# thourihan/DeepfakeDetection

Hardware: AMD Instinct MI355X
Metric: train images/sec @224^2 (EfficientNet-B0) (higher is better)
Workload: dtype bf16; 1 GPU; EfficientNet-b0 (timm flavour) 224x224 train step: bf16 fwd + label-smoothed CE + bwd + AdamW, random-init weights, 2 classes; per_gpu_batch=256, global_batch=256, parallelism=dp1, launch=hipgraph

## Files before the change

deepfakedetection_amd/_lib.py:

```python

from __future__ import annotations

import ctypes
from ctypes import POINTER, Structure, c_double, c_float, c_int, c_int64, c_long, c_size_t, c_uint32, c_void_p
from pathlib import Path

import os as _os

LIB_PATH = Path(_os.environ.get("DFD_LIB_PATH") or Path(__file__).resolve().parent / "libdfd_hip.so")

DFD_OK = 0
ERRORS = {-1: "DFD_EINVAL", -2: "DFD_EUNSUPPORTED", -3: "DFD_ELAUNCH", -4: "DFD_EWORKSPACE"}
F32, BF16 = 0, 1
ACT_NONE, ACT_SILU, ACT_RELU, ACT_GELU = 0, 1, 2, 3
PRO_NONE, PRO_BN_ACT, PRO_BN_ACT_GATE, PRO_AFFINE2 = 0, 1, 2, 3
MAX_PARTIALS = 1024
ADAMW_TABLE_COLS = 5
ADAMW_HP_LEN = 8
EMA_TABLE_COLS = 4
EMA_LERP, EMA_COPY = 0, 1
MIX_JOB_WORDS = 8
MIX_KEEP, MIX_MIXUP, MIX_CUTMIX = 0, 1, 2
MIX_NHWC, MIX_NCHW = 0, 1
AUG_MAX_OPS = 4
# ... 63 lines not shown
    "dfd_pwconv_bwd_fused": (c_int, [c_int, P, P, P, P, P, P, c_int, c_int, c_int, P, P, c_int, P, c_size_t, P]),
    "dfd_pw_prep_weights": (c_int, [c_int, P, P, P, c_int, c_int, P]),
    "dfd_stem_conv_fwd": (c_int, [c_int, P, P, P, POINTER(StemShape), P, c_int, _PI, P]),
    "dfd_stem_conv_wgrad": (c_int, [c_int, P, P, P, P, P, POINTER(StemShape), c_int, P, c_size_t, P]),
    "dfd_stem_conv_wgrad_ws": (c_size_t, [POINTER(StemShape)]),
    "dfd_dropout": (c_int, [P, P, c_float, P, c_int, P]),
    "dfd_linear_fwd": (c_int, [P, P, P, P, c_int, c_int, c_int, P]),
    "dfd_linear_bwd": (c_int, [P, P, P, P, P, P, c_int, c_int, c_int, c_int, P]),
    "dfd_ce_loss": (c_int, [P, P, c_int, c_int, c_float, c_float, P, P, P, P]),
    "dfd_softmax_argmax": (c_int, [P, c_int, c_int, P, P, P]),
    "dfd_adamw_step": (c_int, [P, c_int, P, P]),
    "dfd_ema_update": (c_int, [P, c_int, P, P]),
    "dfd_mix_batch": (c_int, [P, P, P, P, c_int, c_int, c_int, c_int, c_int, P]),
    "dfd_ce_loss_soft": (c_int, [P, P, c_int, c_int, c_float, c_float, P, P, P, P]),
    "dfd_augment_policy_u8": (c_int, [P, P, P, P, c_int, c_int, c_int, P]),
    "dfd_bn_eval_coeffs_multi": (c_int, [P, c_int, P]),
    "dfd_sum_batch_begin": (c_int, []),
    "dfd_sum_batch_end": (c_int, []),
    "dfd_sum_batch_end_deferred": (c_int, []),
    "dfd_sum_passengers_flush": (c_int, [P]),
    "dfd_sum_passengers_discard": (c_int, []),
    "dfd_se_fwd": (c_int, [c_int, P, P, c_int, c_int, c_int, c_int, P, P, P, P, c_int, c_int, P, P, P, P, P, c_size_t, P]),
    "dfd_se_bwd": (c_int, [c_int, P, P, P, c_int, c_int, c_int, c_int, P, P, P, P, P, c_int, c_int, P, P, P, P, P, P, c_int,
                           P, c_size_t, P, P]),
    "dfd_pwconv_fwd_eval": (c_int, [c_int, P, P, P, c_int, P, c_int, c_int, c_int, P]),
    "dfd_dwconv_fwd_eval_tiles": (c_int, [c_int, P]),
    "dfd_dwconv_fwd_eval": (c_int, [c_int, P, P, P, c_int, P, P, P, P, P]),
    "dfd_se_fwd_parts": (c_int, [P, c_int, c_int, c_int, c_int, P, P, P, P, c_int, c_int, P, P, P, P, P]),
    "dfd_bn_finalize_ex": (c_int, [P, c_int, c_int, c_double, P, P, P, P, P, P, c_float, c_float, P, P]),
    "dfd_bn_eval_coeffs_ex": (c_int, [P, P, P, P, P, P, c_float, c_int, P, P]),
# ... 120 lines not shown
```

deepfakedetection_amd/build.py:

```python

from __future__ import annotations

import os
import shutil
import subprocess
import sys
from concurrent.futures import ThreadPoolExecutor
from pathlib import Path

PKG_DIR = Path(__file__).resolve().parent
CSRC = PKG_DIR / "csrc"
OBJ_DIR = CSRC / "build"
LIB_PATH = PKG_DIR / "libdfd_hip.so"
SOURCES = ("dfd_rowpass.hip", "dfd_dwfwd.hip", "dfd_dwbwd.hip", "dfd_dwbwdf.hip", "dfd_dwconv.hip", "dfd_dwmm.hip", "dfd_pwconv.hip", "dfd_pwntw.hip", "dfd_pwntd.hip", "dfd_pwtnw.hip", "dfd_misc.hip", "dfd_vit.hip",
           "dfd_mx.hip", "dfd_attn.hip", "dfd_coord.hip", "dfd_resize.hip", "dfd_augment.hip", "dfd_conv3.hip", "dfd_stem.hip", "dfd_gemm.hip", "dfd_cam.hip", "dfd_mix.hip")
ARCH = "gfx950"
FLAGS = ("-O3", "-fPIC", "-std=c++17", "-ffp-contract=off", f"--offload-arch={ARCH}")


def _hipcc() -> str:
    found = shutil.which("hipcc") or "/opt/rocm/bin/hipcc"
    if not Path(found).exists():
        raise RuntimeError("hipcc not found: libdfd_hip.so cannot be built")
    return found


def _deps_mtime() -> float:
    headers = list(CSRC.glob("*.h")) + [PKG_DIR.parent / "include" / "dfd_hip.h"]
    return max(p.stat().st_mtime for p in headers)
# ... 49 lines not shown
```

deepfakedetection_amd/csrc/dfd_common.h:

```cpp
#pragma once
#include <hip/hip_runtime.h>
#include <stdint.h>
#include <mutex>
#include "../../include/dfd_hip.h"

#define DFD_THREADS 256

template <typename Tag, typename KernelT>
static inline void dfd_allow_lds_once(KernelT kern, int bytes) {
    static std::once_flag once;
    std::call_once(once, [&] { (void)hipFuncSetAttribute(reinterpret_cast<const void*>(kern), hipFuncAttributeMaxDynamicSharedMemorySize, bytes); });
}
template <typename Tag, typename KernelT>
static inline int dfd_kernel_regs_once(KernelT kern, int fallback) {
    static std::once_flag once;
    static int regs = 0;
    std::call_once(once, [&] {
        hipFuncAttributes attr;
        regs = (hipFuncGetAttributes(&attr, reinterpret_cast<const void*>(kern)) == hipSuccess && attr.numRegs > 0) ? attr.numRegs : fallback;
    });
    return regs;
}

struct bf16 { unsigned short x; };
// ... 203 lines not shown
int dfd_stem_wgrad_mfma(const float* x, const void* dz, const void* yraw, const float* coef, const dfd_stem_shape* s, float* ws,
                        int max_rows, int* rows, hipStream_t st);

#define DFD_CHECK_LAUNCH() (hipGetLastError() == hipSuccess ? DFD_OK : DFD_ELAUNCH)

#define DISPATCH_ACT(ACTV, ...)                                                      \
    switch (ACTV) {                                                                  \
        case DFD_ACT_NONE: { constexpr int ACT = DFD_ACT_NONE; __VA_ARGS__; } break; \
        case DFD_ACT_SILU: { constexpr int ACT = DFD_ACT_SILU; __VA_ARGS__; } break; \
        case DFD_ACT_RELU: { constexpr int ACT = DFD_ACT_RELU; __VA_ARGS__; } break; \
        case DFD_ACT_GELU: { constexpr int ACT = DFD_ACT_GELU; __VA_ARGS__; } break; \
        default: return DFD_EUNSUPPORTED;                                            \
    }

enum { DFD_TUNE_DW_MFMA = 0, DFD_TUNE_DW_LDS_KB = 1, DFD_TUNE_DW_GRID = 2, DFD_TUNE_DEBUG = 3, DFD_TUNE_PW_NTD = 4, DFD_TUNE_NTD_NS = 5, DFD_TUNE_NTD_MAXN = 6, DFD_TUNE_NTD_MINT = 7,
       DFD_TUNE_DWQ_GRID_FWD = 8, DFD_TUNE_DWQ_GRID_BWD = 9, DFD_TUNE_DWQ_GRID_WGRAD = 10, DFD_TUNE_DWQ_GRID_MIN = 11, DFD_TUNE_TN_WGS = 12, DFD_TUNE_DWQ_WIDE = 13,
       DFD_TUNE_COUNT = 16 };
int dfd_tune_get(int key);

int dfd_launch_sum_partials(float* partials, int P, long L, float* out, int accumulate, hipStream_t st, bool deferrable = true);
```

deepfakedetection_amd/csrc/dfd_dwmm.hip:

```cpp
#include "dfd_dwm.h"
#include <climits>

typedef float dwm_f4 __attribute__((ext_vector_type(4)));
typedef __bf16 dwm_bf8 __attribute__((ext_vector_type(8)));

static int g_tune[DFD_TUNE_COUNT] = { 1,  156,  256,  0,  1,  0,  0,  16,
                                       1024,  1024,  1024,  32,  512,  -1};
int dfd_tune_get(int key) { return (key >= 0 && key < DFD_TUNE_COUNT) ? g_tune[key] : 0; }
extern "C" int dfd_tune(int key, int value) {
    if (key < 0 || key >= DFD_TUNE_COUNT) return DFD_EINVAL;
    g_tune[key] = value;
    return DFD_OK;
}

#define DWP_THREADS 512
#define DWP_MAXV 6
#define DWP_MAXS 4
#define DWP_MAXR 8

template <int K, int S, int ACT, bool PRO, bool STATS, bool WHOLE>
__global__ void __launch_bounds__(DWP_THREADS, 2)
k_dw_fwd_mp(const unsigned short* __restrict__ x, const float* __restrict__ bnstate, const float* __restrict__ w,
            unsigned short* __restrict__ y, DwMGeom g, float* __restrict__ partials, int dbg) {
    constexpr int KK = K * K, NPAIR = (KK + 1) / 2;
// ... 415 lines not shown
```

deepfakedetection_amd/csrc/dfd_misc.hip:

```cpp
#include "dfd_common.h"
#include "dfd_se.h"

__device__ __forceinline__ float wave_sum(float v) {
#pragma unroll
    for (int o = 32; o >= 1; o >>= 1) v += __shfl_xor(v, o);
    return v;
}
__device__ __forceinline__ float wave_max(float v) {
#pragma unroll
    for (int o = 32; o >= 1; o >>= 1) v = fmaxf(v, __shfl_xor(v, o));
    return v;
}
template <int ACT> __device__ __forceinline__ float act_rt(float z) { return act_fwd<ACT>(z); }

#define SE_MAX_C 4096
#define SE_MAX_R 128

__device__ __forceinline__ float wave_dot(const float* __restrict__ a, const float* __restrict__ b, int C, int lane) {
    float s = 0.f;
    for (int c = lane * 4; c < C; c += 256) {
        const float4 x = *reinterpret_cast<const float4*>(a + c);
        const float4 y = *reinterpret_cast<const float4*>(b + c);
        s = fmaf(x.x, y.x, fmaf(x.y, y.y, fmaf(x.z, y.z, fmaf(x.w, y.w, s))));
    }
// ... 266 lines not shown
                          const float* gate, const float* hpre, const float* pooled, const float* w1, const float* w2t, int R,
                          int act, float* dgate, float* dpooled, float* dw1, float* db1, float* dw2, float* db2, int accumulate,
                          void* pool_ws, size_t pool_ws_bytes, float* ws, dfd_stream stream) {
    if (!D || !y || !bnstate || !gate || !hpre || !pooled || !w1 || !w2t || !dgate || !dpooled || !ws || N < 1 || C < 1 ||
        R < 1 || C % 4)
        return DFD_EINVAL;
    if (C > SE_MAX_C || R > SE_MAX_R) return DFD_EUNSUPPORTED;
    hipStream_t st = (hipStream_t)stream;
    int splits = 1;
    float mul = 1.f;
    const int rc = dfd_pool_launch(dtype, true, D, y, bnstate, act_in, dgate, N, HW, C, pool_ws, pool_ws_bytes, st, &splits, &mul);
    if (rc != DFD_OK) return rc;
    DISPATCH_ACT(act, {
        hipLaunchKernelGGL((k_se_bwd_img<ACT>), dim3(N), dim3(SE_IMG_THREADS), 0, st, (const float*)pool_ws, splits, dgate, gate, hpre,
                           w1, w2t, N, C, R, ws, dpooled);
    });
    if (hipGetLastError() != hipSuccess) return DFD_ELAUNCH;
    if (dw1 && dw2) {
        hipLaunchKernelGGL(k_se_fc_bwd_w, dim3((C + 63) / 64, R), dim3(DFD_THREADS), 0, st, pooled, ws, N, C, R, dw1, db1,
                           dw2, db2, accumulate);
    }
    return DFD_CHECK_LAUNCH();
}

extern "C" int dfd_se_fc_bwd(const float* dgate, const float* gate, const float* hpre, const float* pooled,
                             const float* w1, const float* w2t, int N, int C, int R, int act, float* dpooled,
                             float* dw1, float* db1, float* dw2, float* db2, int accumulate, float* ws,
                             dfd_stream stream) {
    if (!dgate || !gate || !hpre || !pooled || !w1 || !w2t || !dpooled || !ws || N < 1 || C < 1 || R < 1) return DFD_EINVAL;
    if (C > SE_MAX_C || R > SE_MAX_R) return DFD_EUNSUPPORTED;
// ... 670 lines not shown
```

deepfakedetection_amd/csrc/dfd_rowpass.hip:

```cpp
#include "dfd_common.h"
#include "dfd_se.h"
#include "dfd_sum.h"

template <typename T, int ACT, bool HAS_RES, bool HAS_RS>
__global__ void __launch_bounds__(DFD_THREADS)
k_bn_act_apply(const T* __restrict__ y, const float* __restrict__ bnstate, const T* __restrict__ res,
               const float* __restrict__ rs, T* __restrict__ out, long total_vec, int CV, int C, long vec_per_img) {
    constexpr int V = Vec<T>::N;
    const long stride = (long)gridDim.x * DFD_THREADS;
    const long first = (long)blockIdx.x * DFD_THREADS + threadIdx.x;
    int cv = (int)(first % CV);
    const int cstep = (int)(stride % CV);
    for (long i = first; i < total_vec; i += stride, cv = cv + cstep >= CV ? cv + cstep - CV : cv + cstep) {
        const int c0 = cv * V;
        float v[V], sc[V], sh[V];
        Vec<T>::load(y + i * V, v);
        load_f32<V>(bnstate + c0, sc);
        load_f32<V>(bnstate + C + c0, sh);
        float r = 1.f;
        if constexpr (HAS_RS) r = rs[i / vec_per_img];
        float q[V];
        if constexpr (HAS_RES) Vec<T>::load(res + i * V, q);
        bn_act_array<ACT, V>(v, sc, sh);
#pragma unroll
// ... 75 lines not shown
                if constexpr (HAS_Y) acc[V + j] += gg * (yv[j] - mean[j]) * rstd[j];
            }
        }
    }
    reduce_rowlanes<2 * V>(acc, red, cm.cvb, cm.rpb, vl, rl, active);
    if (rl == 0) {
        float* p = partials + (long)blockIdx.x * (HAS_Y ? 2 : 1) * C;
        float a0[V], a1[V];
#pragma unroll
        for (int j = 0; j < V; ++j) { a0[j] = acc[j]; a1[j] = acc[V + j]; }
        store_f32<V>(p + c0, a0);
        if constexpr (HAS_Y) store_f32<V>(p + C + c0, a1);
    }
}

struct SeWgradJob { const float* pooled; const float* ws; int N, C, R; float* dw1; float* db1; float* dw2; float* db2; int accumulate; };

template <typename T, int ACT, int MODE>
__global__ void __launch_bounds__(DFD_THREADS)
k_act_bn_bwd(const T* __restrict__ D, const T* __restrict__ y, const float* __restrict__ gate,
             const float* __restrict__ dpool, const float* __restrict__ bnstate, T* __restrict__ dz,
             long rows, int HW, int C, float invHW, ChanMap cm, float* __restrict__ partials, int main_x, SeWgradJob job,
             SumJobs sum1, SumJobs sum2) {
    constexpr int V = Vec<T>::N;
    __shared__ float red[DFD_THREADS * 2 * V];
    if ((int)blockIdx.x >= main_x) {
        int id = ((int)blockIdx.x - main_x) * (int)gridDim.y + (int)blockIdx.y;
        const int cb = (job.C + 63) / 64, nse = job.dw1 ? cb * job.R : 0;
        if (id < nse) {
            se_fc_bwd_w_body(job.pooled, job.ws, job.N, job.C, job.R, job.dw1, job.db1, job.dw2, job.db2, job.accumulate, id % cb, id / cb, red);
            return;
// ... 561 lines not shown
                                      dfd_stream stream) {
    if (!partials || nparts < 1 || C < 1 || count <= 0 || !bnstate || !coef) return DFD_EINVAL;
    if (dls && (!ls_gamma || !beta)) return DFD_EINVAL;
    const int threads = FIN_CH * FIN_LANES, grid = (C + FIN_CH - 1) / FIN_CH;
    hipLaunchKernelGGL(k_bn_bwd_finalize, dim3(grid), dim3(threads), 0, (hipStream_t)stream, partials, nparts, C, count,
                       gamma, beta, ls_gamma, bnstate, train, dgamma, dbeta, dls, dbias, accumulate, coef);
    return DFD_CHECK_LAUNCH();
}
extern "C" int dfd_bn_bwd_finalize(const float* partials, int nparts, int C, double count, const float* gamma,
                                   const float* bnstate, int train, float* dgamma, float* dbeta, int accumulate,
                                   float* coef, dfd_stream stream) {
    return dfd_bn_bwd_finalize_ex(partials, nparts, C, count, gamma, nullptr, nullptr, bnstate, train, dgamma, dbeta, nullptr,
                                  nullptr, accumulate, coef, stream);
}

extern "C" int dfd_version(void) { return 139; }
```

deepfakedetection_amd/csrc/dfd_se.h:

```cpp
#pragma once
#include "dfd_common.h"

__device__ __forceinline__ float se_wave_sum(float v) {
#pragma unroll
    for (int o = 32; o > 0; o >>= 1) v += __shfl_xor(v, o);
    return v;
}

__device__ __forceinline__ void se_fc_bwd_w_body(const float* __restrict__ pooled, const float* __restrict__ ws, int N, int C, int R,
                                                 float* __restrict__ dw1, float* __restrict__ db1, float* __restrict__ dw2,
                                                 float* __restrict__ db2, int accumulate, int bx, int by, float* red) {
    const float* ws_g = ws;
    const float* ws_dh = ws + (long)N * C;
    const float* ws_h = ws_dh + (long)N * R;
    const int t = threadIdx.x, cl = t & 63, nl = t >> 6;
    const int c = bx * 64 + cl, r = by;
    float a1 = 0.f, a2 = 0.f, sb2 = 0.f;
    if (c < C) {
        int n = nl;
        for (; n + 12 < N; n += 16) {
            float g[4], pc[4], h[4], dh[4];
#pragma unroll
            for (int u = 0; u < 4; ++u) {
                const long m = n + 4 * u;
// ... 21 lines not shown
        if (r == 0 && db2) {
            sb2 = red[(2 * 4 + 0) * 64 + cl] + red[(2 * 4 + 1) * 64 + cl] + red[(2 * 4 + 2) * 64 + cl] + red[(2 * 4 + 3) * 64 + cl];
            db2[c] = (accumulate ? db2[c] : 0.f) + sb2;
        }
    }
    if (bx == 0 && db1) {
        __syncthreads();
        float s = 0.f;
        for (int n = t; n < N; n += DFD_THREADS) s += ws_dh[(long)n * R + r];
        s = se_wave_sum(s);
        if ((t & 63) == 0) red[t >> 6] = s;
        __syncthreads();
        if (t == 0) db1[r] = (accumulate ? db1[r] : 0.f) + red[0] + red[1] + red[2] + red[3];
    }
}
```

deepfakedetection_amd/functions.py:

```python

from __future__ import annotations

import contextlib
import os
import threading
from dataclasses import dataclass

import torch

from . import kernels as K
from ._lib import ACT_NONE, ACT_SILU
from .arch import ConvGeom
from .arena import grad_dest


@dataclass
class BNRef:

    running_mean: torch.Tensor
    running_var: torch.Tensor
    num_batches_tracked: torch.Tensor | None
    momentum: float
    eps: float
    pre: torch.Tensor | None = None
# ... 196 lines not shown
        _, Ho, Wo, Cmid = y2.shape
        with K.sum_batch():
            return MBConvFunction._backward(ctx, g, cfg, x, y1, y2, y3, st1, st2, st3, pooled, hpre, gate, wexp_kn, wproj_kn,
                                            w_dw, w1, w2t, g_exp, g_dw, g_proj, row_scale, need, tr, geom, N, H, W, Cin, Ho, Wo, Cmid)

    @staticmethod
    def _backward(ctx, g, cfg, x, y1, y2, y3, st1, st2, st3, pooled, hpre, gate, wexp_kn, wproj_kn, w_dw, w1, w2t, g_exp, g_dw,
                  g_proj, row_scale, need, tr, geom, N, H, W, Cin, Ho, Wo, Cmid):
        g = _c(g)
        gb = K.scale_rows(g, row_scale) if ctx.has_rs else g
        parts, n = K.bn_bwd_reduce(gb, y3, st3, None)
        Cout, R = y3.shape[3], w1.shape[0]
        coef3, dg_proj, db_proj = K.bn_bwd_finalize(parts, n, N * Ho * Wo, g_proj, st3, tr, need[12] or need[13],
                                                    _dest(ctx, 12, (Cout,)), _dest(ctx, 13, (Cout,)))
        gm3 = K.affine2_apply(gb, y3, coef3)
        D, _, _ = K.pwconv(gm3, None, wproj_kn, None, stats=False)
        dw_proj = None
        if need[11]:
            pro_q = K.pro_bn_act_gate(st2, ACT_SILU, gate, Ho * Wo)
            with K.side_stream(N * Ho * Wo):
                dw_proj = K.pwconv_wgrad(gm3, None, y2, pro_q, _dest(ctx, 11, (Cout, Cmid))).view(Cout, Cmid, 1, 1)
        want_se = need[7] or need[8] or need[9] or need[10]
        se_outs = (_dest(ctx, 7, (R, Cmid)), _dest(ctx, 8, (R,)), _dest(ctx, 9, (Cmid, R)), _dest(ctx, 10, (Cmid,)))
        se_res = K.se_bwd(D, y2, st2, ACT_SILU, gate, hpre, pooled, w1, w2t, ACT_SILU, want_se, se_outs, defer_wgrad=SE_WGRAD_PASSENGER)
        dpooled, dw1, db1, dw2, db2 = se_res[:5]
        se_job = se_res[5] if SE_WGRAD_PASSENGER else None
        dz2, parts, n = K.act_bn_bwd(D, y2, gate, dpooled, st2, ACT_SILU, se_job=se_job)
        if dw1 is not None:
            dw1, dw2 = dw1.view(dw1.shape[0], -1, 1, 1), dw2.view(dw2.shape[0], -1, 1, 1)
        coef2, dg_dw, db_dw = K.bn_bwd_finalize(parts, n, N * Ho * Wo, g_dw, st2, tr, need[5] or need[6],
                                                _dest(ctx, 5, (Cmid,)), _dest(ctx, 6, (Cmid,)))
        kk = geom.kernel
        dw_dw = dx = dw_exp = dg_exp = db_exp = None
        if cfg.expand:
            fused = need[4] and K.dwconv_bwd_fused_ok(geom.kernel, geom.stride)
            if fused:
                dz1, parts, n, dw_dw = K.dwconv_bwd_fused(dz2, y2, coef2, w_dw, y1, st1, ACT_SILU, geom.kernel, geom.stride,
                                                          geom.pad_lead, geom.pad_lead, _dest(ctx, 4, (Cmid, 1, kk, kk)))
            else:
                dz1, parts, n = K.dwconv_bwd_data(dz2, y2, coef2, w_dw, y1, st1, ACT_SILU, y1.shape, geom.kernel,
                                                  geom.stride, geom.pad_lead, geom.pad_lead)
            coef1, dg_exp, db_exp = K.bn_bwd_finalize(parts, n, N * H * W, g_exp, st1, tr, need[2] or need[3],
# ... 149 lines not shown
```

deepfakedetection_amd/kernels.py:

```python

from __future__ import annotations

import contextlib
import functools
import ctypes
import threading
import weakref
from dataclasses import dataclass

import os

import torch

from . import _lib
from ._lib import (
    ACT_NONE, ACT_SILU, BF16, F32, MAX_PARTIALS, MIX_CUTMIX, MIX_JOB_WORDS, MIX_KEEP, MIX_NCHW, MIX_NHWC, PRO_AFFINE2, PRO_BN_ACT,
    PRO_BN_ACT_GATE, PRO_NONE, DwShape, Prologue, StemShape, check,
)

_scratch: dict[tuple[int, int, str], torch.Tensor] = {}


def _L():
    return _lib.load()
# ... 534 lines not shown
        dw2 = _dst(outs[2], (C, R), dev)
        db2 = _dst(outs[3], (C,), dev)
    else:
        dw1 = db1 = dw2 = db2 = None
    pws = _pool_workspace(y, N, H * W, C)
    defer = defer_wgrad and want_param_grads
    check(_L().dfd_se_bwd(_dt(y), _p(D), _p(y), _p(state), act_in, N, H * W, C, _p(gate), _p(hpre), _p(pooled), _p(w1), _p(w2t),
                          R, act, _p(dgate), _p(dpooled), None if defer else _p(dw1), None if defer else _p(db1),
                          None if defer else _p(dw2), None if defer else _p(db2), 0, _p(pws), _nbytes(pws), _p(ws),
                          _stream()), "dfd_se_bwd")
    if defer_wgrad:
        return dpooled, dw1, db1, dw2, db2, ((pooled, ws, R, dw1, db1, dw2, db2) if defer else None)
    return dpooled, dw1, db1, dw2, db2


def _dw_shape(x_shape, Ho: int, Wo: int, k: int, stride: int, pad_top: int, pad_left: int) -> DwShape:
    N, H, W, C = x_shape
    return DwShape(N, H, W, C, Ho, Wo, k, stride, pad_top, pad_left)


def dwconv_fwd(x: torch.Tensor, in_state: torch.Tensor | None, in_act: int, w: torch.Tensor, k: int, stride: int,
               pad_top: int, pad_left: int, Ho: int, Wo: int, stats: bool = True):
    _chk_nhwc(x)
    N, H, W, C = x.shape
    y = torch.empty((N, Ho, Wo, C), dtype=x.dtype, device=x.device)
    shp = _dw_shape(x.shape, Ho, Wo, k, stride, pad_top, pad_left)
    parts = partials_buf(x.device, C) if stats else None
    n = ctypes.c_int(0)
    check(_L().dfd_dwconv_fwd(_dt(x), _p(x), _p(in_state), in_act, _p(w), _p(y), ctypes.byref(shp), _p(parts),
                              MAX_PARTIALS, ctypes.byref(n), _stream()), "dfd_dwconv_fwd", f"{tuple(x.shape)} k{k}s{stride}")
# ... 967 lines not shown
        check(_L().dfd_rand(_p(self.state), stream_id, keep, _p(out), n, _stream()), "dfd_rand")
        return out

    def tick(self, counters: list[torch.Tensor]) -> None:
        key = tuple(c.data_ptr() for c in counters)
        if key != self._counter_key:
            self._counter_key = key
            with torch.inference_mode(False):
                self._counter_table = torch.tensor(list(key), dtype=torch.int64).to(self.state.device) if key else None
        journal_note(counters)
        check(_L().dfd_step_tick(_p(self._counter_table), len(key), _p(self.state), _stream()), "dfd_step_tick")


_profile_sink: list | None = None
_TIMED = ("bn_act_apply", "bn_bwd_reduce", "act_bn_bwd", "pool_act", "pool_bwd_reduce", "scale_rows", "dwconv_fwd",
          "dwconv_bwd_data", "dwconv_bwd_weight", "dwconv_bwd_fused", "pwconv", "pwconv_wgrad", "pwconv_bwd_fused", "stem_conv_fwd", "stem_conv_wgrad",
          "se_fc_fwd", "se_fc_bwd", "linear_fwd", "linear_bwd", "ce_loss", "adamw_step", "prep_weights", "bn_finalize",
          "bn_bwd_finalize", "bn_bwd_finalize_ex", "dropout", "bgemm", "attn_scores", "attn_apply", "attn_softmax_fwd", "attn_softmax_bwd", "im2col", "col2im",
          "wattn_fwd", "wattn_bwd", "mx_quant_rows", "mx_gemm",
          "bn_add_act", "bn_add_act_bwd", "affine2_apply", "up2_act_fwd", "up2_act_bwd", "layernorm_fwd", "layernorm_bwd",
          "channel_stats", "subsample_add")


def set_profile_sink(sink: list | None) -> None:
    global _profile_sink
    _profile_sink = sink


def _tensor_bytes(obj) -> int:
    if isinstance(obj, torch.Tensor):
        if obj.dim() <= 1 and obj.numel() >= MAX_PARTIALS:
# ... 78 lines not shown
```

include/dfd_hip.h:

```cpp
#ifndef DFD_HIP_H
#define DFD_HIP_H

#include <stddef.h>
#include <stdint.h>

#ifdef __cplusplus
extern "C" {
#endif

typedef void* dfd_stream;

#define DFD_OK            0
#define DFD_EINVAL       (-1)
#define DFD_EUNSUPPORTED (-2)
#define DFD_ELAUNCH      (-3)
#define DFD_EWORKSPACE   (-4)

#define DFD_F32   0
#define DFD_BF16  1

#define DFD_ACT_NONE 0
#define DFD_ACT_SILU 1
#define DFD_ACT_RELU 2
#define DFD_ACT_GELU 3
// ... 54 lines not shown
int dfd_gemm_bias_act(int dtype, const void* a, const void* w_nk, int M, int K, int N, const float* state, int act,
                      const void* residual, const float* row_scale, int HW, void* yraw, void* out, dfd_stream stream);
int dfd_gemm_plan(int M, int K, int N);
int dfd_pw_ntd_plan(int M, int K, int Nout);
size_t dfd_bias_grad_ws(int N, int HW, int C);
int dfd_bias_grad(int dtype, const void* g, const float* row_scale, int N, int HW, int C, float* dbias, int accumulate,
                  float* ws, size_t ws_bytes, dfd_stream stream);
int dfd_act_bn_bwd(int dtype, const void* D, const void* y, const float* gate,
                   const float* dpool, const float* bnstate, int act, void* dz,
                   int N, int HW, int C, float* partials, int pcap, int* nparts,
                   dfd_stream stream);
int dfd_act_bn_bwd_se(int dtype, const void* D, const void* y, const float* gate, const float* dpool,
                      const float* bnstate, int act, void* dz, int N, int HW, int C, float* partials, int pcap,
                      int* nparts, const float* se_pooled, const float* se_ws, int R, float* dw1, float* db1, float* dw2,
                      float* db2, int accumulate, dfd_stream stream);
size_t dfd_pool_ws(int dtype, int N, int HW, int C);
int dfd_pool_act(int dtype, const void* y, const float* bnstate, int act, float* pooled,
                 int N, int HW, int C, void* ws, size_t ws_bytes, dfd_stream stream);
int dfd_pool_bwd_reduce(int dtype, const void* D, const void* y, const float* bnstate,
                        int act, float* dgate, int N, int HW, int C, void* ws, size_t ws_bytes,
                        dfd_stream stream);
int dfd_scale_rows(int dtype, const void* x, const float* row_scale, void* out,
                   int N, int HW, int C, dfd_stream stream);

int dfd_se_fc_fwd(const float* pooled, const float* w1, const float* b1, const float* w2,
                  const float* b2, int N, int C, int R, int act, float* hpre, float* gate,
                  float* w2t, dfd_stream stream);
int dfd_se_fc_bwd(const float* dgate, const float* gate, const float* hpre,
                  const float* pooled, const float* w1, const float* w2t,
                  int N, int C, int R, int act, float* dpooled,
                  float* dw1, float* db1, float* dw2, float* db2, int accumulate,
                  float* ws, dfd_stream stream);
int dfd_se_fwd(int dtype, const void* y, const float* bnstate, int act_in, int N, int HW, int C,
               const float* w1, const float* b1, const float* w2, const float* b2, int R, int act,
               float* pooled, float* hpre, float* gate, float* w2t, void* ws, size_t ws_bytes,
               dfd_stream stream);
int dfd_se_bwd(int dtype, const void* D, const void* y, const float* bnstate, int act_in, int N, int HW,
               int C, const float* gate, const float* hpre, const float* pooled, const float* w1,
               const float* w2t, int R, int act, float* dgate, float* dpooled, float* dw1, float* db1,
               float* dw2, float* db2, int accumulate, void* pool_ws, size_t pool_ws_bytes, float* ws,
               dfd_stream stream);

typedef struct {
    int N, H, W, C;
    int Ho, Wo;
    int k, stride, pad_top, pad_left;
} dfd_dwconv_shape;

int dfd_dwconv_fwd(int dtype, const void* x, const float* in_bnstate, int in_act,
                   const float* w, void* y, const dfd_dwconv_shape* s,
                   float* partials, int pcap, int* nparts, dfd_stream stream);
int dfd_dwconv_bwd_data(int dtype, const void* dz, const void* y, const float* coef,
                        const float* w, const void* xin, const float* in_bnstate, int in_act,
                        void* dzin, const dfd_dwconv_shape* s,
                        float* partials, int pcap, int* nparts, dfd_stream stream);
int dfd_dwconv_bwd_weight(int dtype, const void* dz, const void* y, const float* coef,
// ... 283 lines not shown
```

Baseline: 20680 images/sec.

## Fuse projection dgrad GEMM into SE gate and act-BN backward kernels

Adds a new kernel that recomputes the projection-conv data gradient (gm3 × Wproj) in registers via MFMA and consumes it directly, instead of materialising D to memory. It runs twice: once to produce per-split gate reduction partials for SE backward, and once fused with the SiLU/BN backward that writes dz and the BN partials. SE weight-grad and sum passenger jobs ride along as extra workgroups. This trades a D write plus two D reads for recomputing the small-K GEMM twice, and is enabled by default only for Cout<=64.

```diff
diff --git a/deepfakedetection_amd/_lib.py b/deepfakedetection_amd/_lib.py
--- a/deepfakedetection_amd/_lib.py
+++ b/deepfakedetection_amd/_lib.py
@@ -101,6 +101,12 @@
     "dfd_mix_batch": (c_int, [P, P, P, P, c_int, c_int, c_int, c_int, c_int, P]),
     "dfd_ce_loss_soft": (c_int, [P, P, c_int, c_int, c_float, c_float, P, P, P, P]),
     "dfd_augment_policy_u8": (c_int, [P, P, P, P, c_int, c_int, c_int, P]),
+    "dfd_proj_bwd_plan": (c_int, [c_int, c_int, c_int, c_int]),
+    "dfd_proj_bwd_gate_ws": (c_size_t, [c_int, c_int, c_int, c_int]),
+    "dfd_proj_bwd_gate": (c_int, [c_int, P, P, P, P, c_int, c_int, c_int, c_int, c_int, P, c_size_t, _PI, P]),
+    "dfd_proj_bwd_act": (c_int, [c_int, P, P, P, P, P, P, c_int, P, c_int, c_int, c_int, c_int, P, c_int, _PI, P, P, c_int, P, P, P, P,
+                                 c_int, P]),
+    "dfd_se_bwd_parts": (c_int, [P, c_int, c_int, c_int, P, P, P, P, P, c_int, c_int, P, P, P, P, P, c_int, P, P]),
     "dfd_bn_eval_coeffs_multi": (c_int, [P, c_int, P]),
     "dfd_sum_batch_begin": (c_int, []),
     "dfd_sum_batch_end": (c_int, []),
diff --git a/deepfakedetection_amd/build.py b/deepfakedetection_amd/build.py
--- a/deepfakedetection_amd/build.py
+++ b/deepfakedetection_amd/build.py
@@ -12,7 +12,7 @@
 CSRC = PKG_DIR / "csrc"
 OBJ_DIR = CSRC / "build"
 LIB_PATH = PKG_DIR / "libdfd_hip.so"
-SOURCES = ("dfd_rowpass.hip", "dfd_dwfwd.hip", "dfd_dwbwd.hip", "dfd_dwbwdf.hip", "dfd_dwconv.hip", "dfd_dwmm.hip", "dfd_pwconv.hip", "dfd_pwntw.hip", "dfd_pwntd.hip", "dfd_pwtnw.hip", "dfd_misc.hip", "dfd_vit.hip",
+SOURCES = ("dfd_rowpass.hip", "dfd_dwfwd.hip", "dfd_dwbwd.hip", "dfd_dwbwdf.hip", "dfd_dwconv.hip", "dfd_dwmm.hip", "dfd_pwconv.hip", "dfd_pwntw.hip", "dfd_pwntd.hip", "dfd_pwtnw.hip", "dfd_projbwd.hip", "dfd_misc.hip", "dfd_vit.hip",
            "dfd_mx.hip", "dfd_attn.hip", "dfd_coord.hip", "dfd_resize.hip", "dfd_augment.hip", "dfd_conv3.hip", "dfd_stem.hip", "dfd_gemm.hip", "dfd_cam.hip", "dfd_mix.hip")
 ARCH = "gfx950"
 FLAGS = ("-O3", "-fPIC", "-std=c++17", "-ffp-contract=off", f"--offload-arch={ARCH}")
diff --git a/deepfakedetection_amd/csrc/dfd_common.h b/deepfakedetection_amd/csrc/dfd_common.h
--- a/deepfakedetection_amd/csrc/dfd_common.h
+++ b/deepfakedetection_amd/csrc/dfd_common.h
@@ -241,7 +241,7 @@
     }
 
 enum { DFD_TUNE_DW_MFMA = 0, DFD_TUNE_DW_LDS_KB = 1, DFD_TUNE_DW_GRID = 2, DFD_TUNE_DEBUG = 3, DFD_TUNE_PW_NTD = 4, DFD_TUNE_NTD_NS = 5, DFD_TUNE_NTD_MAXN = 6, DFD_TUNE_NTD_MINT = 7,
-       DFD_TUNE_DWQ_GRID_FWD = 8, DFD_TUNE_DWQ_GRID_BWD = 9, DFD_TUNE_DWQ_GRID_WGRAD = 10, DFD_TUNE_DWQ_GRID_MIN = 11, DFD_TUNE_TN_WGS = 12, DFD_TUNE_DWQ_WIDE = 13,
+       DFD_TUNE_DWQ_GRID_FWD = 8, DFD_TUNE_DWQ_GRID_BWD = 9, DFD_TUNE_DWQ_GRID_WGRAD = 10, DFD_TUNE_DWQ_GRID_MIN = 11, DFD_TUNE_TN_WGS = 12, DFD_TUNE_DWQ_WIDE = 13, DFD_TUNE_PROJ_BWD = 14,
        DFD_TUNE_COUNT = 16 };
 int dfd_tune_get(int key);
 
diff --git a/deepfakedetection_amd/csrc/dfd_dwmm.hip b/deepfakedetection_amd/csrc/dfd_dwmm.hip
--- a/deepfakedetection_amd/csrc/dfd_dwmm.hip
+++ b/deepfakedetection_amd/csrc/dfd_dwmm.hip
@@ -5,7 +5,7 @@
 typedef __bf16 dwm_bf8 __attribute__((ext_vector_type(8)));
 
 static int g_tune[DFD_TUNE_COUNT] = { 1,  156,  256,  0,  1,  0,  0,  16,
-                                       1024,  1024,  1024,  32,  512,  -1};
+                                       1024,  1024,  1024,  32,  512,  -1,  1};
 int dfd_tune_get(int key) { return (key >= 0 && key < DFD_TUNE_COUNT) ? g_tune[key] : 0; }
 extern "C" int dfd_tune(int key, int value) {
     if (key < 0 || key >= DFD_TUNE_COUNT) return DFD_EINVAL;
diff --git a/deepfakedetection_amd/csrc/dfd_misc.hip b/deepfakedetection_amd/csrc/dfd_misc.hip
--- a/deepfakedetection_amd/csrc/dfd_misc.hip
+++ b/deepfakedetection_amd/csrc/dfd_misc.hip
@@ -304,6 +304,25 @@
     DISPATCH_ACT(act, {
         hipLaunchKernelGGL((k_se_bwd_img<ACT>), dim3(N), dim3(SE_IMG_THREADS), 0, st, (const float*)pool_ws, splits, dgate, gate, hpre,
                            w1, w2t, N, C, R, ws, dpooled);
+    });
+    if (hipGetLastError() != hipSuccess) return DFD_ELAUNCH;
+    if (dw1 && dw2) {
+        hipLaunchKernelGGL(k_se_fc_bwd_w, dim3((C + 63) / 64, R), dim3(DFD_THREADS), 0, st, pooled, ws, N, C, R, dw1, db1,
+                           dw2, db2, accumulate);
+    }
+    return DFD_CHECK_LAUNCH();
+}
+
+extern "C" int dfd_se_bwd_parts(const float* parts, int splits, int N, int C, const float* gate, const float* hpre,
+                                const float* pooled, const float* w1, const float* w2t, int R, int act, float* dpooled, float* dw1,
+                                float* db1, float* dw2, float* db2, int accumulate, float* ws, dfd_stream stream) {
+    if (!parts || splits < 1 || !gate || !hpre || !pooled || !w1 || !w2t || !dpooled || !ws || N < 1 || C < 1 || R < 1 || C % 4)
+        return DFD_EINVAL;
+    if (C > SE_MAX_C || R > SE_MAX_R) return DFD_EUNSUPPORTED;
+    hipStream_t st = (hipStream_t)stream;
+    DISPATCH_ACT(act, {
+        hipLaunchKernelGGL((k_se_bwd_img<ACT>), dim3(N), dim3(SE_IMG_THREADS), 0, st, parts, splits, parts, gate, hpre, w1, w2t, N, C,
+                           R, ws, dpooled);
     });
     if (hipGetLastError() != hipSuccess) return DFD_ELAUNCH;
     if (dw1 && dw2) {
diff --git a/deepfakedetection_amd/csrc/dfd_projbwd.hip b/deepfakedetection_amd/csrc/dfd_projbwd.hip
--- /dev/null
+++ b/deepfakedetection_amd/csrc/dfd_projbwd.hip
@@ -0,0 +1,315 @@
+#include "dfd_pw.h"
+#include "dfd_se.h"
+#include "dfd_sum.h"
+
+#define PB_WAVES (MODE == 0 ? (BN == 32 ? 4 : 3) : (BN == 32 ? 3 : 2))
+template <int BN, int KSN, int MODE, int ACT>
+__global__ void __launch_bounds__(DFD_THREADS, PB_WAVES)
+k_proj_bwd(const bf16* __restrict__ gm, const bf16* __restrict__ w, const bf16* __restrict__ y, const float* __restrict__ bnstate,
+           const float* __restrict__ gate, const float* __restrict__ dpool, bf16* __restrict__ dz, float* __restrict__ out,
+           int N, int HW, int K, int C, int n_tiles, int splits, int rows_per, float invHW, int main_wgs, SeWgradJob job,
+           SumJobs sum1, SumJobs sum2) {
+    using T = bf16;
+    constexpr int E = 8;
+    constexpr int JN = 2;
+    constexpr int WR = 16 * JN;
+    constexpr int BM = 4 * WR;
+    constexpr int NT = BN / 16;
+    constexpr int WSTRIDE = KSN * 64 + 16;
+    constexpr int OROW = BN * 2 + 16;
+    constexpr int CPR = BN / E;
+    constexpr int RL = 64 / CPR;
+    constexpr int NPS = WR / RL;
+    constexpr int NV = MODE == 0 ? E : 2 * E;
+    extern __shared__ __attribute__((aligned(16))) unsigned char smem[];
+
+    if ((int)blockIdx.x >= main_wgs) {
+        if constexpr (MODE == 1) {
+            int id = (int)blockIdx.x - main_wgs;
+            const int cb = (job.C + 63) / 64, nse = job.dw1 ? cb * job.R : 0;
+            if (id < nse) {
+                se_fc_bwd_w_body(job.pooled, job.ws, job.N, job.C, job.R, job.dw1, job.db1, job.dw2, job.db2, job.accumulate, id % cb,
+                                 id / cb, reinterpret_cast<float*>(smem));
+                return;
+            }
+            id -= nse;
+            const int n1 = sum1.n > 0 ? sum1.gx * sum1.gofs[sum1.n] : 0;
+            if (id < n1) { sum_multi_body(sum1, 1, id % sum1.gx, id / sum1.gx); return; }
+            id -= n1;
+            if (sum2.n > 0 && id < sum2.gx * sum2.n) sum_multi_body(sum2, 2, id % sum2.gx, id / sum2.gx);
+        }
+        return;
+    }
+    int lin = blockIdx.x;
+    {
+        const int q = main_wgs >> 3, r = main_wgs & 7, xcd = lin & 7, slot = lin >> 3;
+        lin = (xcd < r ? xcd * (q + 1) : r * (q + 1) + (xcd - r) * q) + slot;
+    }
+    const int nt = lin % n_tiles, rest = lin / n_tiles;
+    const int z = rest % splits, n = rest / splits;
+    const int n0 = nt * BN;
+    const int r_beg = z * rows_per;
+    const int r_end = r_beg + rows_per < HW ? r_beg + rows_per : HW;
+    const int tiles = (r_end - r_beg + BM - 1) / BM;
+    const int t = threadIdx.x, lane = t & 63, wave = t >> 6;
+    const int frow = lane & 15, fk = lane >> 4;
+    const bf16* gmb = gm + (long)n * HW * K;
+    const bf16* yb = y + (long)n * HW * C;
+
+    for (int idx = t; idx < BN * KSN * 4; idx += DFD_THREADS) {
+        const int nn = idx / (KSN * 4), c = idx - nn * (KSN * 4);
+        uint4 v = make_uint4(0, 0, 0, 0);
+        if (n0 + nn < C && c * E < K) v = *reinterpret_cast<const uint4*>(w + (long)(n0 + nn) * K + c * E);
+        *reinterpret_cast<uint4*>(smem + nn * WSTRIDE + c * 16) = v;
+    }
+
+    const int ec = lane % CPR, er = lane / CPR;
+    const int nch = n0 + ec * E;
+    const bool valid = nch < C;
+    const int ncl = valid ? nch : 0;
+    float sc[E], sh[E], mean[E], gt[E], dp[E];
+    load_f32<E>(bnstate + ncl, sc);
+    load_f32<E>(bnstate + C + ncl, sh);
+    if constexpr (MODE == 1) {
+        load_f32<E>(bnstate + 2 * C + ncl, mean);
+        load_f32<E>(gate + (long)n * C + ncl, gt);
+        load_f32<E>(dpool + (long)n * C + ncl, dp);
+#pragma unroll
+        for (int j = 0; j < E; ++j) dp[j] = dp[j] * invHW;
+    }
+    float acc[NV];
+#pragma unroll
+    for (int j = 0; j < NV; ++j) acc[j] = 0.f;
+    __syncthreads();
+
+    uint4 R0[JN][KSN], R1[JN][KSN], Y0[NPS], Y1[NPS];
+    auto g_load = [&](uint4 (&R)[JN][KSN], int i) {
+        const int rbase = r_beg + i * BM + wave * WR + frow;
+#pragma unroll
+        for (int j = 0; j < JN; ++j)
+#pragma unroll
+            for (int ks = 0; ks < KSN; ++ks) {
+                const int row = rbase + j * 16, kk = (ks * 4 + fk) * E;
+                R[j][ks] = *reinterpret_cast<const uint4*>(gmb + (long)(row < r_end ? row : r_end - 1) * K + (kk < K ? kk : 0));
+            }
+    };
+    auto y_load = [&](uint4 (&Y)[NPS], int i) {
+        const int rbase = r_beg + i * BM + wave * WR + er;
+#pragma unroll
+        for (int p = 0; p < NPS; ++p) {
+            const int row = rbase + p * RL;
+            Y[p] = *reinterpret_cast<const uint4*>(yb + (long)(row < r_end ? row : r_end - 1) * C + ncl);
+        }
+    };
+    f32x4_t cacc[NT][JN];
+#pragma unroll
+    for (int i = 0; i < NT; ++i)
+#pragma unroll
+        for (int j = 0; j < JN; ++j) cacc[i][j] = (f32x4_t){0.f, 0.f, 0.f, 0.f};
+    unsigned char* eb = smem + BN * WSTRIDE + wave * WR * OROW;
+
+    auto step = [&](uint4 (&rcur)[JN][KSN], uint4 (&rnext)[JN][KSN], uint4 (&ycur)[NPS], uint4 (&ynext)[NPS], int i) {
+        uint4 fa[JN][KSN];
+#pragma unroll
+        for (int j = 0; j < JN; ++j)
+#pragma unroll
+            for (int ks = 0; ks < KSN; ++ks) fa[j][ks] = ((ks * 4 + fk) * E < K) ? rcur[j][ks] : make_uint4(0, 0, 0, 0);
+        if (i + 1 < tiles) {
+            g_load(rnext, i + 1);
+            y_load(ynext, i + 1);
+        }
+        const int mw = r_beg + i * BM + wave * WR;
+        {
+            const unsigned char* wbase = smem + frow * WSTRIDE + fk * 16;
+#pragma unroll
+            for (int ks = 0; ks < KSN; ++ks) {
+                if (ks * 4 * E < K) {
+#pragma unroll
+                    for (int ii = 0; ii < NT; ++ii) {
+                        const uint4 fw = *reinterpret_cast<const uint4*>(wbase + ks * 64 + ii * 16 * WSTRIDE);
+#pragma unroll
+                        for (int j = 0; j < JN; ++j)
+                            cacc[ii][j] = __builtin_amdgcn_mfma_f32_16x16x32_bf16(__builtin_bit_cast(bf16x8_t, fw),
+                                                                                 __builtin_bit_cast(bf16x8_t, fa[j][ks]), cacc[ii][j], 0, 0, 0);
+                    }
+                }
+            }
+        }
+#pragma unroll
+        for (int ii = 0; ii < NT; ++ii)
+#pragma unroll
+            for (int j = 0; j < JN; ++j) {
+                uint2 q;
+                q.x = pack_bf2(cacc[ii][j][0], cacc[ii][j][1]);
+                q.y = pack_bf2(cacc[ii][j][2], cacc[ii][j][3]);
+                *reinterpret_cast<uint2*>(eb + (j * 16 + frow) * OROW + (ii * 16 + fk * 4) * 2) = q;
+                cacc[ii][j] = (f32x4_t){0.f, 0.f, 0.f, 0.f};
+            }
+        __builtin_amdgcn_fence(__ATOMIC_RELEASE, "wavefront");
+        __builtin_amdgcn_wave_barrier();
+        __builtin_amdgcn_fence(__ATOMIC_ACQUIRE, "wavefront");
+#pragma unroll
+        for (int p = 0; p < NPS; ++p) {
+            const int rr = er + p * RL;
+            const int m = mw + rr;
+            float dv[E], yv[E];
+            q_to_f(*reinterpret_cast<const uint4*>(eb + rr * OROW + ec * 16), dv);
+            q_to_f(ycur[p], yv);
+            if constexpr (MODE == 0) {
+                float a0[E];
+#pragma unroll
+                for (int j = 0; j < E; ++j) a0[j] = yv[j];
+                bn_act_array<ACT, E>(a0, sc, sh);
+                if (m < r_end) {
+#pragma unroll
+                    for (int j = 0; j < E; ++j) acc[j] += round_to<T>(a0[j]) * dv[j];
+                }
+            } else {
+                float agr[E];
+#pragma unroll
+                for (int j = 0; j < E; j += 2) {
+                    const dfd_f2 z2 = __builtin_elementwise_fma((dfd_f2){sc[j], sc[j + 1]}, (dfd_f2){yv[j], yv[j + 1]}, (dfd_f2){sh[j], sh[j + 1]});
+                    const dfd_f2 g2 = act_grad2<ACT>(z2);
+                    agr[j] = g2.x; agr[j + 1] = g2.y;
+                }
+                if (m < r_end && valid) {
+#pragma unroll
+                    for (int j = 0; j < E; ++j) {
+                        const float da = fmaf(dv[j], gt[j], dp[j]);
+                        const float d = round_to<T>(da * agr[j]);
+                        dv[j] = d;
+                        acc[j] += d;
+                        acc[E + j] += d * (yv[j] - mean[j]);
+                    }
+                    Vec<T>::store(dz + ((long)n * HW + m) * C + nch, dv);
+                }
+            }
+        }
+        __builtin_amdgcn_fence(__ATOMIC_RELEASE, "wavefront");
+        __builtin_amdgcn_wave_barrier();
+        __builtin_amdgcn_fence(__ATOMIC_ACQUIRE, "wavefront");
+    };
+
+    g_load(R0, 0);
+    y_load(Y0, 0);
+    for (int i = 0; i < tiles; i += 2) {
+        step(R0, R1, Y0, Y1, i);
+        if (i + 1 < tiles) step(R1, R0, Y1, Y0, i + 1);
+    }
+
+    __syncthreads();
+    float* red = reinterpret_cast<float*>(smem);
+    const int rl = t / CPR;
+    reduce_rowlanes<NV>(acc, red, CPR, DFD_THREADS / CPR, ec, rl, true);
+    if (rl == 0 && valid) {
+        if constexpr (MODE == 0) {
+            store_f32<E>(out + ((long)z * N + n) * C + nch, acc);
+        } else {
+            float* p = out + (long)(n * splits + z) * 2 * C;
+            float a0[E], a1[E], rstd[E];
+            load_f32<E>(bnstate + 3 * C + nch, rstd);
+#pragma unroll
+            for (int j = 0; j < E; ++j) { a0[j] = acc[j]; a1[j] = acc[E + j] * rstd[j]; }
+            store_f32<E>(p + nch, a0);
+            store_f32<E>(p + C + nch, a1);
+        }
+    }
+}
+
+struct ProjBwdPlan { int bn, ksn, n_tiles, splits, rows_per, lds; };
+
+static ProjBwdPlan proj_bwd_plan(int N, int HW, int K, int C, int max_parts) {
+    ProjBwdPlan p{0, 0, 0, 0, 0, 0};
+    if (!(dfd_tune_get(DFD_TUNE_PROJ_BWD) & 1)) return p;
+    if (N < 1 || HW < 1 || K < 8 || C < 8 || K % 8 || C % 8 || K > 64) return p;
+    if (max_parts > DFD_MAX_PARTIALS) max_parts = DFD_MAX_PARTIALS;
+    if (N > max_parts || (long)N * HW >= (1l << 31)) return p;
+    p.ksn = K <= 32 ? 1 : 2;
+    p.bn = C <= 32 ? 32 : 64;
+    const int BM = 128;
+    p.n_tiles = (C + p.bn - 1) / p.bn;
+    int s = 1024 / (N * p.n_tiles);
+    if (s > HW / (2 * BM)) s = HW / (2 * BM);
+    if (s > 32) s = 32;
+    if (s > max_parts / N) s = max_parts / N;
+    if (s < 1) s = 1;
+    int rp = (HW + s - 1) / s;
+    if (s > 1) rp = (rp + BM - 1) / BM * BM;
+    p.splits = (HW + rp - 1) / rp;
+    p.rows_per = rp;
+    const int wstride = p.ksn * 64 + 16, orow = p.bn * 2 + 16;
+    p.lds = p.bn * wstride + 4 * 32 * orow;
+    if (p.lds < DFD_THREADS * 2 * 8 * 4) p.lds = DFD_THREADS * 2 * 8 * 4;
+    return p;
+}
+
+extern "C" int dfd_proj_bwd_plan(int N, int HW, int Cout, int Cmid) { return proj_bwd_plan(N, HW, Cout, Cmid, DFD_MAX_PARTIALS).bn; }
+
+extern "C" size_t dfd_proj_bwd_gate_ws(int N, int HW, int Cout, int Cmid) {
+    const ProjBwdPlan p = proj_bwd_plan(N, HW, Cout, Cmid, DFD_MAX_PARTIALS);
+    return p.bn ? (size_t)p.splits * N * Cmid * sizeof(float) : 0;
+}
+
+template <int MODE>
+static int proj_bwd_launch(const ProjBwdPlan& p, const void* gm3, const void* w_kn, const void* y, const float* bnstate,
+                           const float* gate, const float* dpool, void* dz, float* out, int N, int HW, int K, int C, int extra,
+                           const SeWgradJob& job, const SumJobs& sum1, const SumJobs& sum2, hipStream_t st) {
+    constexpr int ACT = DFD_ACT_SILU;
+    const int main_wgs = p.n_tiles * N * p.splits;
+    const float invHW = 1.0f / (float)HW;
+#define LAUNCH_PB(BN, KSN)                                                                                                        \
+    hipLaunchKernelGGL((k_proj_bwd<BN, KSN, MODE, ACT>), dim3(main_wgs + extra), dim3(DFD_THREADS), p.lds, st, (const bf16*)gm3,   \
+                       (const bf16*)w_kn, (const bf16*)y, bnstate, gate, dpool, (bf16*)dz, out, N, HW, K, C, p.n_tiles, p.splits,  \
+                       p.rows_per, invHW, main_wgs, job, sum1, sum2)
+    if (p.bn == 32 && p.ksn == 1) LAUNCH_PB(32, 1);
+    else if (p.bn == 64 && p.ksn == 1) LAUNCH_PB(64, 1);
+    else if (p.bn == 32) LAUNCH_PB(32, 2);
+    else LAUNCH_PB(64, 2);
+#undef LAUNCH_PB
+    return DFD_CHECK_LAUNCH();
+}
+
+extern "C" int dfd_proj_bwd_gate(int dtype, const void* gm3, const void* w_kn, const void* y, const float* bnstate, int act, int N,
+                                 int HW, int Cout, int Cmid, float* parts, size_t parts_bytes, int* splits, dfd_stream stream) {
+    if (!gm3 || !w_kn || !y || !bnstate || !parts || !splits || N < 1 || HW < 1 || Cout < 1 || Cmid < 1) return DFD_EINVAL;
+    if (dtype != DFD_BF16 || act != DFD_ACT_SILU) return DFD_EUNSUPPORTED;
+    const ProjBwdPlan p = proj_bwd_plan(N, HW, Cout, Cmid, DFD_MAX_PARTIALS);
+    if (!p.bn) return DFD_EUNSUPPORTED;
+    if (parts_bytes < (size_t)p.splits * N * Cmid * sizeof(float)) return DFD_EWORKSPACE;
+    *splits = p.splits;
+    SumJobs none;
+    none.n = 0;
+    const SeWgradJob job{nullptr, nullptr, 0, 0, 0, nullptr, nullptr, nullptr, nullptr, 0};
+    return proj_bwd_launch<0>(p, gm3, w_kn, y, bnstate, nullptr, nullptr, nullptr, parts, N, HW, Cout, Cmid, 0, job, none, none,
+                              (hipStream_t)stream);
+}
+
+extern "C" int dfd_proj_bwd_act(int dtype, const void* gm3, const void* w_kn, const void* y, const float* gate, const float* dpool,
+                                const float* bnstate, int act, void* dz, int N, int HW, int Cout, int Cmid, float* partials, int pcap,
+                                int* nparts, const float* se_pooled, const float* se_ws, int R, float* dw1, float* db1, float* dw2,
+                                float* db2, int accumulate, dfd_stream stream) {
+    if (!gm3 || !w_kn || !y || !gate || !dpool || !bnstate || !dz || !partials || !nparts || pcap < 1 || N < 1 || HW < 1 ||
+        Cout < 1 || Cmid < 1)
+        return DFD_EINVAL;
+    const bool se = se_pooled || se_ws || dw1 || dw2;
+    if (se && (!se_pooled || !se_ws || !dw1 || !dw2 || R < 1)) return DFD_EINVAL;
+    if (dtype != DFD_BF16 || act != DFD_ACT_SILU) return DFD_EUNSUPPORTED;
+    const ProjBwdPlan p = proj_bwd_plan(N, HW, Cout, Cmid, pcap);
+    if (!p.bn) return DFD_EUNSUPPORTED;
+    hipStream_t st = (hipStream_t)stream;
+    SeWgradJob job{nullptr, nullptr, 0, 0, 0, nullptr, nullptr, nullptr, nullptr, 0};
+    SumJobs sum1, sum2;
+    dfd_sum_passengers_take(st, &sum1, &sum2);
+    long passengers = (sum1.n > 0 ? (long)sum1.gx * sum1.gofs[sum1.n] : 0) + (sum2.n > 0 ? (long)sum2.gx * sum2.n : 0);
+    if (se) {
+        job = SeWgradJob{se_pooled, se_ws, N, Cmid, R, dw1, db1, dw2, db2, accumulate};
+        passengers += (long)((Cmid + 63) / 64) * R;
+    }
+    *nparts = N * p.splits;
+    if (proj_bwd_launch<1>(p, gm3, w_kn, y, bnstate, gate, dpool, dz, partials, N, HW, Cout, Cmid, (int)passengers, job, sum1, sum2,
+                           st) != DFD_OK) {
+        dfd_sum_passengers_untake(st, &sum1, &sum2);
+        return DFD_ELAUNCH;
+    }
+    return DFD_OK;
+}
diff --git a/deepfakedetection_amd/csrc/dfd_rowpass.hip b/deepfakedetection_amd/csrc/dfd_rowpass.hip
--- a/deepfakedetection_amd/csrc/dfd_rowpass.hip
+++ b/deepfakedetection_amd/csrc/dfd_rowpass.hip
@@ -113,7 +113,6 @@
     }
 }
 
-struct SeWgradJob { const float* pooled; const float* ws; int N, C, R; float* dw1; float* db1; float* dw2; float* db2; int accumulate; };
 
 template <typename T, int ACT, int MODE>
 __global__ void __launch_bounds__(DFD_THREADS)
@@ -705,4 +704,4 @@
                                   nullptr, accumulate, coef, stream);
 }
 
-extern "C" int dfd_version(void) { return 139; }
+extern "C" int dfd_version(void) { return 140; }
diff --git a/deepfakedetection_amd/csrc/dfd_se.h b/deepfakedetection_amd/csrc/dfd_se.h
--- a/deepfakedetection_amd/csrc/dfd_se.h
+++ b/deepfakedetection_amd/csrc/dfd_se.h
@@ -59,3 +59,5 @@
         if (t == 0) db1[r] = (accumulate ? db1[r] : 0.f) + red[0] + red[1] + red[2] + red[3];
     }
 }
+
+struct SeWgradJob { const float* pooled; const float* ws; int N, C, R; float* dw1; float* db1; float* dw2; float* db2; int accumulate; };
diff --git a/deepfakedetection_amd/functions.py b/deepfakedetection_amd/functions.py
--- a/deepfakedetection_amd/functions.py
+++ b/deepfakedetection_amd/functions.py
@@ -234,7 +234,8 @@
         coef3, dg_proj, db_proj = K.bn_bwd_finalize(parts, n, N * Ho * Wo, g_proj, st3, tr, need[12] or need[13],
                                                     _dest(ctx, 12, (Cout,)), _dest(ctx, 13, (Cout,)))
         gm3 = K.affine2_apply(gb, y3, coef3)
-        D, _, _ = K.pwconv(gm3, None, wproj_kn, None, stats=False)
+        fused_d = K.proj_bwd_ok(gm3, y2)
+        D = None if fused_d else K.pwconv(gm3, None, wproj_kn, None, stats=False)[0]
         dw_proj = None
         if need[11]:
             pro_q = K.pro_bn_act_gate(st2, ACT_SILU, gate, Ho * Wo)
@@ -242,10 +243,19 @@
                 dw_proj = K.pwconv_wgrad(gm3, None, y2, pro_q, _dest(ctx, 11, (Cout, Cmid))).view(Cout, Cmid, 1, 1)
         want_se = need[7] or need[8] or need[9] or need[10]
         se_outs = (_dest(ctx, 7, (R, Cmid)), _dest(ctx, 8, (R,)), _dest(ctx, 9, (Cmid, R)), _dest(ctx, 10, (Cmid,)))
-        se_res = K.se_bwd(D, y2, st2, ACT_SILU, gate, hpre, pooled, w1, w2t, ACT_SILU, want_se, se_outs, defer_wgrad=SE_WGRAD_PASSENGER)
+        if fused_d:
+            gparts, gsplits = K.proj_bwd_gate(gm3, wproj_kn, y2, st2, ACT_SILU)
+            se_res = K.se_bwd_parts(gparts, gsplits, gate, hpre, pooled, w1, w2t, ACT_SILU, want_se, se_outs,
+                                    defer_wgrad=SE_WGRAD_PASSENGER)
+        else:
+            se_res = K.se_bwd(D, y2, st2, ACT_SILU, gate, hpre, pooled, w1, w2t, ACT_SILU, want_se, se_outs,
+                              defer_wgrad=SE_WGRAD_PASSENGER)
         dpooled, dw1, db1, dw2, db2 = se_res[:5]
         se_job = se_res[5] if SE_WGRAD_PASSENGER else None
-        dz2, parts, n = K.act_bn_bwd(D, y2, gate, dpooled, st2, ACT_SILU, se_job=se_job)
+        if fused_d:
+            dz2, parts, n = K.proj_bwd_act(gm3, wproj_kn, y2, gate, dpooled, st2, ACT_SILU, se_job=se_job)
+        else:
+            dz2, parts, n = K.act_bn_bwd(D, y2, gate, dpooled, st2, ACT_SILU, se_job=se_job)
         if dw1 is not None:
             dw1, dw2 = dw1.view(dw1.shape[0], -1, 1, 1), dw2.view(dw2.shape[0], -1, 1, 1)
         coef2, dg_dw, db_dw = K.bn_bwd_finalize(parts, n, N * Ho * Wo, g_dw, st2, tr, need[5] or need[6],
diff --git a/deepfakedetection_amd/kernels.py b/deepfakedetection_amd/kernels.py
--- a/deepfakedetection_amd/kernels.py
+++ b/deepfakedetection_amd/kernels.py
@@ -572,6 +572,65 @@
     return dpooled, dw1, db1, dw2, db2
 
 
+def proj_bwd_ok(gm3: torch.Tensor, y: torch.Tensor) -> bool:
+    if y.dtype != torch.bfloat16 or gm3.dtype != torch.bfloat16:
+        return False
+    N, H, W, C = y.shape
+    return int(_L().dfd_proj_bwd_plan(N, H * W, gm3.shape[-1], C)) != 0
+
+
+def proj_bwd_gate(gm3: torch.Tensor, w_kn: torch.Tensor, y: torch.Tensor, state: torch.Tensor, act: int):
+    _chk_nhwc(y)
+    N, H, W, C = y.shape
+    Cout = gm3.shape[-1]
+    nbytes = int(_L().dfd_proj_bwd_gate_ws(N, H * W, Cout, C))
+    parts = scratch(y.device, "proj_gate_parts", nbytes)
+    splits = ctypes.c_int(0)
+    check(_L().dfd_proj_bwd_gate(_dt(y), _p(gm3), _p(w_kn), _p(y), _p(state), act, N, H * W, Cout, C, _p(parts), nbytes,
+                                 ctypes.byref(splits), _stream()), "dfd_proj_bwd_gate", f"{tuple(y.shape)} Cout={Cout}")
+    return parts, splits.value
+
+
+def se_bwd_parts(parts: torch.Tensor, splits: int, gate, hpre, pooled, w1, w2t, act: int, want_param_grads: bool = True,
+                 outs=(None, None, None, None), defer_wgrad: bool = False):
+    N, C = pooled.shape
+    R = w1.shape[0]
+    dev = pooled.device
+    dpooled = torch.empty((N, C), dtype=torch.float32, device=dev)
+    ws = scratch(dev, "se_ws", (N * C + 2 * N * R) * 4)
+    if want_param_grads:
+        dw1 = _dst(outs[0], (R, C), dev)
+        db1 = _dst(outs[1], (R,), dev)
+        dw2 = _dst(outs[2], (C, R), dev)
+        db2 = _dst(outs[3], (C,), dev)
+    else:
+        dw1 = db1 = dw2 = db2 = None
+    defer = defer_wgrad and want_param_grads
+    check(_L().dfd_se_bwd_parts(_p(parts), splits, N, C, _p(gate), _p(hpre), _p(pooled), _p(w1), _p(w2t), R, act, _p(dpooled),
+                                None if defer else _p(dw1), None if defer else _p(db1), None if defer else _p(dw2),
+                                None if defer else _p(db2), 0, _p(ws), _stream()), "dfd_se_bwd_parts")
+    if defer_wgrad:
+        return dpooled, dw1, db1, dw2, db2, ((pooled, ws, R, dw1, db1, dw2, db2) if defer else None)
+    return dpooled, dw1, db1, dw2, db2
+
+
+def proj_bwd_act(gm3: torch.Tensor, w_kn: torch.Tensor, y: torch.Tensor, gate: torch.Tensor, dpool: torch.Tensor,
+                 state: torch.Tensor, act: int, se_job: tuple | None = None):
+    _chk_nhwc(y)
+    N, H, W, C = y.shape
+    Cout = gm3.shape[-1]
+    if _passenger_task is not None and torch._C._current_graph_task_id() != _passenger_task:
+        drop_passengers()
+    dz = torch.empty_like(y)
+    parts = partials_buf(y.device, C)
+    n = ctypes.c_int(0)
+    pooled, ws, R, dw1, db1, dw2, db2 = se_job if se_job is not None else (None, None, 0, None, None, None, None)
+    check(_L().dfd_proj_bwd_act(_dt(y), _p(gm3), _p(w_kn), _p(y), _p(gate), _p(dpool), _p(state), act, _p(dz), N, H * W, Cout, C,
+                                _p(parts), MAX_PARTIALS, ctypes.byref(n), _p(pooled), _p(ws), R, _p(dw1), _p(db1), _p(dw2), _p(db2),
+                                0, _stream()), "dfd_proj_bwd_act", f"{tuple(y.shape)} Cout={Cout}")
+    return dz, parts, n.value
+
+
 def _dw_shape(x_shape, Ho: int, Wo: int, k: int, stride: int, pad_top: int, pad_left: int) -> DwShape:
     N, H, W, C = x_shape
     return DwShape(N, H, W, C, Ho, Wo, k, stride, pad_top, pad_left)
@@ -1569,7 +1628,7 @@
 
 _profile_sink: list | None = None
 _TIMED = ("bn_act_apply", "bn_bwd_reduce", "act_bn_bwd", "pool_act", "pool_bwd_reduce", "scale_rows", "dwconv_fwd",
-          "dwconv_bwd_data", "dwconv_bwd_weight", "dwconv_bwd_fused", "pwconv", "pwconv_wgrad", "pwconv_bwd_fused", "stem_conv_fwd", "stem_conv_wgrad",
+          "dwconv_bwd_data", "dwconv_bwd_weight", "dwconv_bwd_fused", "pwconv", "pwconv_wgrad", "pwconv_bwd_fused", "proj_bwd_gate", "proj_bwd_act", "stem_conv_fwd", "stem_conv_wgrad",
           "se_fc_fwd", "se_fc_bwd", "linear_fwd", "linear_bwd", "ce_loss", "adamw_step", "prep_weights", "bn_finalize",
           "bn_bwd_finalize", "bn_bwd_finalize_ex", "dropout", "bgemm", "attn_scores", "attn_apply", "attn_softmax_fwd", "attn_softmax_bwd", "im2col", "col2im",
           "wattn_fwd", "wattn_bwd", "mx_quant_rows", "mx_gemm",
diff --git a/include/dfd_hip.h b/include/dfd_hip.h
--- a/include/dfd_hip.h
+++ b/include/dfd_hip.h
@@ -92,6 +92,14 @@
                       const float* bnstate, int act, void* dz, int N, int HW, int C, float* partials, int pcap,
                       int* nparts, const float* se_pooled, const float* se_ws, int R, float* dw1, float* db1, float* dw2,
                       float* db2, int accumulate, dfd_stream stream);
+int dfd_proj_bwd_plan(int N, int HW, int Cout, int Cmid);
+size_t dfd_proj_bwd_gate_ws(int N, int HW, int Cout, int Cmid);
+int dfd_proj_bwd_gate(int dtype, const void* gm3, const void* w_kn, const void* y, const float* bnstate, int act, int N, int HW,
+                      int Cout, int Cmid, float* parts, size_t parts_bytes, int* splits, dfd_stream stream);
+int dfd_proj_bwd_act(int dtype, const void* gm3, const void* w_kn, const void* y, const float* gate, const float* dpool,
+                     const float* bnstate, int act, void* dz, int N, int HW, int Cout, int Cmid, float* partials, int pcap,
+                     int* nparts, const float* se_pooled, const float* se_ws, int R, float* dw1, float* db1, float* dw2, float* db2,
+                     int accumulate, dfd_stream stream);
 size_t dfd_pool_ws(int dtype, int N, int HW, int C);
 int dfd_pool_act(int dtype, const void* y, const float* bnstate, int act, float* pooled,
                  int N, int HW, int C, void* ws, size_t ws_bytes, dfd_stream stream);
@@ -118,6 +126,9 @@
                const float* w2t, int R, int act, float* dgate, float* dpooled, float* dw1, float* db1,
                float* dw2, float* db2, int accumulate, void* pool_ws, size_t pool_ws_bytes, float* ws,
                dfd_stream stream);
+int dfd_se_bwd_parts(const float* parts, int splits, int N, int C, const float* gate, const float* hpre, const float* pooled,
+                     const float* w1, const float* w2t, int R, int act, float* dpooled, float* dw1, float* db1, float* dw2,
+                     float* db2, int accumulate, float* ws, dfd_stream stream);
 
 typedef struct {
     int N, H, W, C;
```

Measured after the change: 21010 images/sec (median of 6 runs). 1.6% higher.
